# riktor/safer2-recommender

Hardware: AMD Instinct MI355X
Metric: user-solve updates/sec + sec/epoch, iALS dim=256 ml20m-shaped (higher is better)
Workload: dtype f32

## Files before the change

### safer2-recommender_amd/csrc/common.h

```cpp
#pragma once

#include <hip/hip_runtime.h>
#include <stdint.h>

#ifdef FRECSYS_ABLATION
#define FRECSYS_SKIP(mask, bit) ((mask) & (bit))
#else
#define FRECSYS_SKIP(mask, bit) 0
#endif

namespace frecsys_hip {

typedef float f32x16 __attribute__((ext_vector_type(16)));

enum {
  KIND_IALS = 0,
  KIND_WEIGHTED_U = 1,
  KIND_WEIGHTED_V = 2,
  KIND_CVAR_GRAD_U = 3,
  KIND_CVAR_GRAD_V = 4,
};

__host__ __device__ __forceinline__ bool is_v_kind(int k) {
  return k == KIND_WEIGHTED_V || k == KIND_CVAR_GRAD_V;
}
__host__ __device__ __forceinline__ bool is_u_kind(int k) {
  return k == KIND_WEIGHTED_U || k == KIND_CVAR_GRAD_U;
}
__host__ __device__ __forceinline__ bool is_grad_kind(int k) {
  return k == KIND_CVAR_GRAD_U || k == KIND_CVAR_GRAD_V;
}

__host__ __device__ constexpr int tidx(int I, int J) { return I * (I + 1) / 2 + J; }

__device__ __forceinline__ int sw(int r, int c) {
  return r * 32 + ((((c >> 2) ^ (r >> 1)) & 7) << 2) + (c & 3);
}
typedef float f32x4v __attribute__((ext_vector_type(4)));
__device__ __forceinline__ f32x4v row_gran(const float* tile, int r, int G) {
  return *reinterpret_cast<const f32x4v*>(tile + r * 32 + (((G ^ (r >> 1)) & 7) << 2));
}

__device__ __forceinline__ int acc_row(int q, int hi) {
  return (q & 3) + 8 * (q >> 2) + 4 * hi;
}

__device__ __forceinline__ void lds_barrier() {
  asm volatile("s_waitcnt lgkmcnt(0)" ::: "memory");
  __builtin_amdgcn_s_barrier();
  asm volatile("" ::: "memory");
}

__device__ __forceinline__ void wave_lds_sync() {
  asm volatile("s_waitcnt lgkmcnt(0)" ::: "memory");
  __builtin_amdgcn_wave_barrier();
  asm volatile("" ::: "memory");
}

__device__ __forceinline__ void glds16(const void* src, unsigned dst) {
  unsigned keep;
  asm volatile(
      "s_mov_b32 %0, m0\n\ts_mov_b32 m0, %2\n\ts_nop 0\n\t"
      "global_load_lds_dwordx4 %1, off\n\ts_mov_b32 m0, %0"
      : "=&s"(keep)
      : "v"(src), "s"(dst)
      : "memory");
}
__device__ __forceinline__ void glds4(const void* src, unsigned dst) {
  unsigned keep;
  asm volatile(
      "s_mov_b32 %0, m0\n\ts_mov_b32 m0, %2\n\ts_nop 0\n\t"
      "global_load_lds_dword %1, off\n\ts_mov_b32 m0, %0"
      : "=&s"(keep)
      : "v"(src), "s"(dst)
      : "memory");
}
__device__ __forceinline__ void vm_wait(int n) {
  switch (__builtin_amdgcn_readfirstlane(n)) {
    case 0: asm volatile("s_waitcnt vmcnt(0)" ::: "memory"); break;
    case 1: asm volatile("s_waitcnt vmcnt(1)" ::: "memory"); break;
    case 2: asm volatile("s_waitcnt vmcnt(2)" ::: "memory"); break;
    case 5: asm volatile("s_waitcnt vmcnt(5)" ::: "memory"); break;
    case 6: asm volatile("s_waitcnt vmcnt(6)" ::: "memory"); break;
    case 7: asm volatile("s_waitcnt vmcnt(7)" ::: "memory"); break;
    case 8: asm volatile("s_waitcnt vmcnt(8)" ::: "memory"); break;
    case 10: asm volatile("s_waitcnt vmcnt(10)" ::: "memory"); break;
    case 24: asm volatile("s_waitcnt vmcnt(24)" ::: "memory"); break;
    case 48: asm volatile("s_waitcnt vmcnt(48)" ::: "memory"); break;
    default: asm volatile("s_waitcnt vmcnt(0)" ::: "memory"); break;
  }
}
__device__ __forceinline__ void w3_barrier() {
  asm volatile("s_waitcnt lgkmcnt(0)" ::: "memory");
  __builtin_amdgcn_s_barrier();
  asm volatile("" ::: "memory");
}

__device__ __forceinline__ unsigned lds_addr(const void* p) {
  return (unsigned)(uintptr_t)(const __attribute__((address_space(3))) char*)p;
}

__device__ __forceinline__ f32x16 mfma32(float a, float b, f32x16 c) {
  return __builtin_amdgcn_mfma_f32_32x32x2f32(a, b, c, 0, 0, 0);
}

__device__ __forceinline__ uint32_t score_key(float x) {
  const uint32_t u = __float_as_uint(x);
  return (u & 0x80000000u) ? ~u : (u | 0x80000000u);
}
__device__ __forceinline__ float score_unkey(uint32_t key) {
  return __uint_as_float((key & 0x80000000u) ? (key ^ 0x80000000u) : ~key);
}

typedef __bf16 bf16x8 __attribute__((ext_vector_type(8)));

__device__ __forceinline__ void split3(float x, __bf16& h, __bf16& m, __bf16& l) {
  h = (__bf16)x;
  float r = x - (float)h;
  m = (__bf16)r;
  r -= (float)m;
  l = (__bf16)r;
}

__device__ __forceinline__ f32x16 mfma_bf16(bf16x8 a, bf16x8 b, f32x16 c) {
  return __builtin_amdgcn_mfma_f32_32x32x16_bf16(a, b, c, 0, 0, 0);
}

__device__ __forceinline__ f32x16 mfma_x6(const bf16x8 (&a)[3], const bf16x8 (&b)[3], f32x16 c) {
  c = mfma_bf16(a[2], b[0], c);
  c = mfma_bf16(a[0], b[2], c);
  c = mfma_bf16(a[1], b[1], c);
  c = mfma_bf16(a[1], b[0], c);
  c = mfma_bf16(a[0], b[1], c);
  c = mfma_bf16(a[0], b[0], c);
  return c;
}

__device__ __forceinline__ f32x16 mfma_x6s(const bf16x8 (&a)[3], const bf16x8 (&b)[3], f32x16 c) {
  c = mfma_bf16(a[0], b[0], c);
  c = mfma_bf16(a[0], b[1], c);
  c = mfma_bf16(a[1], b[0], c);
  c = mfma_bf16(a[0], b[2], c);
  c = mfma_bf16(a[1], b[1], c);
  c = mfma_bf16(a[2], b[0], c);
  return c;
}

__device__ __forceinline__ void split3x8(const float (&x)[8], bf16x8 (&f)[3]) {
#pragma unroll
  for (int j = 0; j < 8; ++j) {
    __bf16 h, m, l;
    split3(x[j], h, m, l);
    f[0][j] = h;
    f[1][j] = m;
    f[2][j] = l;
  }
}

__device__ __forceinline__ float entity_lambda(int kind, float reg, float reg_exp, float w,
                                               float alpha, int64_t h, int64_t n_other,
                                               const float* entity_reg, int64_t e,
// ... 107 lines not shown
```

### safer2-recommender_amd/csrc/dual.hip

```cpp
#include <hip/hip_runtime.h>

#include <cstdlib>
#include <type_traits>

#include "chol.h"
#include "common.h"
#include "kernels.h"

namespace frecsys_hip {

namespace {

constexpr int kMaxDp = 1024;

template <int HP>
__device__ __forceinline__ int dgran(int p, int g, int hh, int j) {
  return ((p * 2 + g) * 2 + hh) * HP + j;
}

template <int TH, bool BF>
struct DualCfg {
  static constexpr int HP = 32 * TH;
  static constexpr int NT = TH * (TH + 1) / 2;
  static constexpr int NW = (TH <= 4) ? 4 : 8;
  static constexpr int NTHR = NW * 64;
  static constexpr int MT = (NT + NW - 1) / NW;
  static constexpr int SROW = 33;
  static constexpr int STG = HP * SROW;
  static constexpr int ZS = (BF ? 48 : 32) * HP;
  static constexpr int TILES = NT * 1024;
  static constexpr int NSTAGE = BF ? 0 : ((TH <= 4) ? 1 : 2);
  static constexpr int NSTG1 = NSTAGE > 0 ? NSTAGE : 1;
  static constexpr int LOOP = ((NSTAGE * STG + ZS + 3) / 4) * 4;
  static constexpr int REGION0 = TILES > LOOP ? TILES : LOOP;
  static constexpr int OFF_C = REGION0;
  static constexpr int OFF_ID = OFF_C + HP;
  static constexpr int OFF_B = OFF_ID + HP;
  static constexpr int OFF_X = OFF_B + HP;
  static constexpr int PART = NTHR > NW * 32 ? NTHR : NW * 32;
  static constexpr int OFF_PART = OFF_X + HP;
  static constexpr int OFF_FLAG = OFF_PART + PART;
  static constexpr int OFF_L = OFF_FLAG + 4;
  static constexpr int NQ = (HP * 8 + NTHR - 1) / NTHR;
  static constexpr int WPE = (TH == 3 || TH == 5) ? 4 : (TH == 4 ? 3 : 1);
  static constexpr size_t bytes(int Dp) { return (size_t)(OFF_L + 2 * Dp) * 4; }
  static_assert(bytes(kMaxDp) <= 163840, "LDS budget");
};

__device__ __forceinline__ int64_t virt_pos_d(int64_t k, int64_t h) {
  return k < h ? k : (h - 128 + (k - h));
}

__device__ __forceinline__ void dual_scalars(const DualArgs& a, int64_t e, int64_t h, float& mu,
                                             float& lam, float& omega) {
  const int kind = a.kind;
  const bool uk = is_u_kind(kind);
  omega = (uk && a.entity_weight) ? a.entity_weight[e] : 1.0f;
  lam = entity_lambda(kind, a.reg, a.reg_exp, a.w, a.alpha, h, a.n_other, a.entity_reg, e,
                      a.lambda_is_reg);
  mu = uk ? omega * a.w : a.w;
}

__global__ void __launch_bounds__(256) dual_ldl_kernel(DualArgs a) {
  __shared__ float td[kMaxDp], to[kMaxDp];
  const int Dp = a.Dp, tid = threadIdx.x;
  if (a.unit_m) {
    const int64_t p = (int64_t)blockIdx.x * 256 + tid;
    if (p >= a.n_rows) return;
    const int64_t pp = a.pos0 + p;
    for (int k = 0; k < Dp; ++k) {
      a.table[blk_t(pp, 0, k, Dp)] = 0.0f;
      a.table[blk_t(pp, 1, k, Dp)] = 1.0f;
      a.table[blk_t(pp, 2, k, Dp)] = 1.0f;
    }
    if (!(a.basis_status[0] > 0.5f)) atomicMin(a.fail, (unsigned long long)(a.order[p].entity + 1));
    return;
  }
  for (int k = tid; k < Dp; k += 256) {
    td[k] = a.tdiag[k];
    to[k] = a.toff[k];
  }
  lds_barrier();
  const int64_t p = (int64_t)blockIdx.x * 256 + tid;
  if (p >= a.n_rows) return;
  const QueueRec rec = a.order[p];
  float mu, lam, omega;
  dual_scalars(a, rec.entity, rec.h, mu, lam, omega);
  const int64_t pp = a.pos0 + p;
  float r = 0.0f;
  bool ok = true;
  for (int k = 0; k < Dp; ++k) {
    const float b = k > 0 ? mu * to[k - 1] : 0.0f;
    const float l = b * r;
    const float dk = (mu * td[k] + lam) - l * b;
    ok = ok && (dk > 0.0f);
    r = __builtin_amdgcn_rcpf(dk);
    a.table[blk_t(pp, 0, k, Dp)] = l;
    a.table[blk_t(pp, 1, k, Dp)] = __builtin_amdgcn_rsqf(dk);
    a.table[blk_t(pp, 2, k, Dp)] = r;
  }
  if (!ok) atomicMin(a.fail, (unsigned long long)(rec.entity + 1));
}

constexpr int SWEEP_CH = 32;
__global__ void __launch_bounds__(256) dual_sweep_kernel(DualArgs a) {
  const int Dp = a.Dp;
  const int64_t p = (int64_t)blockIdx.x * 256 + threadIdx.x;
  if (p >= a.n_rows) return;
  const int64_t pp = a.pos0 + p;
  float u = 0.0f;
  for (int k0 = 0; k0 < Dp; k0 += SWEEP_CH) {
    float vv[SWEEP_CH], ll[SWEEP_CH], dd[SWEEP_CH];
#pragma unroll
    for (int j = 0; j < SWEEP_CH; ++j) {
      vv[j] = a.out_rot[blk_v(pp, k0 + j, Dp)];
      ll[j] = a.table[blk_t(pp, 0, k0 + j, Dp)];
      dd[j] = a.table[blk_t(pp, 2, k0 + j, Dp)];
    }
#pragma unroll
    for (int j = 0; j < SWEEP_CH; ++j) {
      u = vv[j] - ll[j] * u;
      a.out_rot[blk_v(pp, k0 + j, Dp)] = u * dd[j];
    }
  }
  float x = 0.0f;
  for (int k1 = Dp; k1 > 0; k1 -= SWEEP_CH) {
    float vv[SWEEP_CH], ll[SWEEP_CH];
#pragma unroll
    for (int j = 0; j < SWEEP_CH; ++j) {
      const int k = k1 - 1 - j;
      vv[j] = a.out_rot[blk_v(pp, k, Dp)];
      ll[j] = k + 1 < Dp ? a.table[blk_t(pp, 0, k + 1, Dp)] : 0.0f;
    }
#pragma unroll
    for (int j = 0; j < SWEEP_CH; ++j) {
      x = vv[j] - ll[j] * x;
      a.out_rot[blk_v(pp, k1 - 1 - j, Dp)] = x;
    }
  }
}

constexpr int kDualBlkTH = 3;

template <int TH, bool BF>
__global__ void __launch_bounds__((DualCfg<TH, BF>::NTHR))
    __attribute__((amdgpu_waves_per_eu(DualCfg<TH, BF>::WPE, 8))) dual_solve_kernel(DualArgs a) {
  using C = DualCfg<TH, BF>;
  constexpr bool RDS = BF;
  constexpr int HP = C::HP, NT = C::NT, NW = C::NW, NTHR = C::NTHR, MT = C::MT;
  constexpr int SROW = C::SROW, NQ = C::NQ;
  extern __shared__ __attribute__((aligned(16))) float smem[];
  float* tiles = smem;
  float* stage = smem;
  float* zs = smem + C::NSTAGE * C::STG;
  float* lsub = smem + C::OFF_L;
  float* dsq = lsub + a.Dp;
  float* cvec = smem + C::OFF_C;
  int* ids = reinterpret_cast<int*>(smem + C::OFF_ID);
  float* bvec = smem + C::OFF_B;
  float* xvec = smem + C::OFF_X;
  float* part = smem + C::OFF_PART;
  int* flag = reinterpret_cast<int*>(smem + C::OFF_FLAG);

  const int tid = threadIdx.x, lane = tid & 63;
  const int wave = __builtin_amdgcn_readfirstlane(tid >> 6);
  const int lo = lane & 31, hi = lane >> 5;
  const int kind = a.kind;
  const bool vk = is_v_kind(kind), uk = is_u_kind(kind);
  const int Dp = a.Dp, NC = Dp >> 5;

  const QueueRec rec = a.order[blockIdx.x];
  const int64_t e = rec.entity;
  const int64_t h = rec.h;
  const int64_t p0 = rec.p0;
  int64_t extra = 0;
  if (vk && a.quirk && h > 128 && (h % 128) != 0) extra = 128 - (h % 128);
  const int ntot = (int)(h + extra);

  const float hf = (float)h;
  float mu, lam, omega;
  dual_scalars(a, e, h, mu, lam, omega);
  (void)mu;
  (void)lam;

  int my_id = -1;
  if (tid < HP) {
    int id = -1;
    float cj = 0.0f;
    if (tid < ntot) {
      id = a.col[p0 + virt_pos_d(tid, h)];
      cj = vk ? sqrtf(a.other_weight[id]) : (uk ? sqrtf(omega / hf) : 1.0f);
    }
    ids[tid] = id;
    cvec[tid] = cj;
    bvec[tid] = tid < h ? cj : 0.0f;
    my_id = id;
  }
  if (tid == 0) flag[0] = 0;
  unsigned long long t_prev = a.prof ? clock64() : 0;
  auto mark = [&](int ph) {
    if (a.prof && tid == 0) {
      const unsigned long long t = clock64();
      atomicAdd(a.prof + ph, t - t_prev);
      t_prev = t;
    }
  };
  {
    const int64_t pp = a.pos0 + blockIdx.x;
    for (int k = tid; k < Dp; k += NTHR) {
      lsub[k] = FRECSYS_SKIP(a.debug_skip, 256) ? 0.5f : a.table[blk_t(pp, 0, k, Dp)];
      dsq[k] = FRECSYS_SKIP(a.debug_skip, 256) ? 0.5f : a.table[blk_t(pp, 1, k, Dp)];
    }
  }
  lds_barrier();

  float4 ra[NQ], rb[NQ];
  auto load_slab = [&](int c, float4 (&regs)[NQ]) {
#pragma unroll
    for (int q = 0; q < NQ; ++q) {
      const int s = tid + q * NTHR;
      if ((HP * 8) % NTHR == 0 || s < HP * 8) {
        const int r = s >> 3, c4 = s & 7;
        const int id = max(ids[r], 0);
        regs[q] = *reinterpret_cast<const float4*>(a.Xrot + (int64_t)id * Dp + 32 * c + 4 * c4);
      }
    }
  };
  auto store_slab = [&](const float4 (&regs)[NQ], int buf) {
#pragma unroll
    for (int q = 0; q < NQ; ++q) {
      const int s = tid + q * NTHR;
      if ((HP * 8) % NTHR == 0 || s < HP * 8) {
        const int r = s >> 3, c4 = s & 7;
        const bool ok = ids[r] >= 0 && !FRECSYS_SKIP(a.debug_skip, 32);
        float* d = stage + (buf % C::NSTG1) * C::STG + r * SROW + 4 * c4;
        d[0] = ok ? regs[q].x : 0.0f;
        d[1] = ok ? regs[q].y : 0.0f;
        d[2] = ok ? regs[q].z : 0.0f;
        d[3] = ok ? regs[q].w : 0.0f;
      }
    }
  };

  const float* myrow = a.Xrot + (int64_t)max(my_id, 0) * Dp;
  float4 yq[RDS ? 8 : 1];
  if constexpr (RDS) {
    if (tid < HP) {
#pragma unroll
      for (int q = 0; q < 8; ++q) yq[q] = *reinterpret_cast<const float4*>(myrow + 4 * q);
    }
  } else {
    load_slab(0, ra);
    if (NC > 1) load_slab(1, rb);
    store_slab(ra, 0);
  }
  lds_barrier();
  mark(0);

  f32x16 acc[MT];
  int aoff[MT], boff[MT];
  bool valid[MT];
#pragma unroll
  for (int m = 0; m < MT; ++m) {
    const int t = wave + m * NW;
    valid[m] = t < NT;
    int I = 0;
    while ((I + 1) * (I + 2) / 2 <= t) ++I;
    const int J = t - I * (I + 1) / 2;
    aoff[m] = 32 * I + lo;
    boff[m] = 32 * J + lo;
    acc[m] = f32x16{0.f};
  }
  float carry = 0.0f;
  const float cj = tid < HP ? cvec[tid] : 0.0f;
  auto slab_step = [&](int c, float4 (&mine)[NQ], float4 (&next)[NQ]) {
    if (!RDS && c + 2 < NC) load_slab(c + 2, mine);
    if (RDS && tid < HP && !FRECSYS_SKIP(a.debug_skip, 128)) {
      bf16x8* zb = reinterpret_cast<bf16x8*>(zs);
      float z = carry;
#pragma unroll
      for (int gh = 0; gh < 4; ++gh) {
        float v[8];
#pragma unroll
        for (int u = 0; u < 8; ++u) {
          const float4 y4 = yq[2 * gh + (u >> 2)];
          const float yv = (u & 3) == 0 ? y4.x : (u & 3) == 1 ? y4.y : (u & 3) == 2 ? y4.z : y4.w;
          const int k = 32 * c + 8 * gh + u;
          z = yv - lsub[k] * z;
          v[u] = (cj * z) * dsq[k];
        }
        if (c + 1 < NC) {
          yq[2 * gh] = *reinterpret_cast<const float4*>(myrow + 32 * (c + 1) + 8 * gh);
          yq[2 * gh + 1] = *reinterpret_cast<const float4*>(myrow + 32 * (c + 1) + 8 * gh + 4);
        }
        bf16x8 f[3];
        split3x8(v, f);
#pragma unroll
        for (int p = 0; p < 3; ++p) zb[dgran<HP>(p, gh >> 1, gh & 1, tid)] = f[p];
      }
      carry = z;
    }
    if (!RDS && tid < HP && !FRECSYS_SKIP(a.debug_skip, 128)) {
      const float* yrow = stage + ((c & 1) % C::NSTG1) * C::STG + tid * SROW;
      float y[BF ? 1 : 32];
      if constexpr (!BF) {
#pragma unroll
        for (int kk = 0; kk < 32; ++kk) y[kk] = yrow[kk];
      }
      float z = carry;
      if constexpr (BF) {
        bf16x8* zb = reinterpret_cast<bf16x8*>(zs);
#pragma unroll
        for (int gh = 0; gh < 4; ++gh) {
          float v[8];
#pragma unroll
          for (int u = 0; u < 8; ++u) {
            const int kk = 8 * gh + u, k = 32 * c + kk;
            z = yrow[kk] - lsub[k] * z;
            v[u] = (cj * z) * dsq[k];
          }
          bf16x8 f[3];
          split3x8(v, f);
#pragma unroll
          for (int p = 0; p < 3; ++p) zb[dgran<HP>(p, gh >> 1, gh & 1, tid)] = f[p];
        }
      } else {
#pragma unroll
        for (int kk = 0; kk < 32; ++kk) {
          const int k = 32 * c + kk;
          z = y[kk] - lsub[k] * z;
          zs[kk * HP + tid] = (cj * z) * dsq[k];
        }
      }
      carry = z;
    }
    lds_barrier();
    if (!FRECSYS_SKIP(a.debug_skip, 1)) {
      if constexpr (BF) {
        const bf16x8* zb = reinterpret_cast<const bf16x8*>(zs);
#pragma unroll
        for (int m = 0; m < MT; ++m) {
          if (valid[m]) {
#pragma unroll
            for (int g = 0; g < 2; ++g) {
              bf16x8 av[3], bv[3];
#pragma unroll
              for (int p = 0; p < 3; ++p) {
                av[p] = zb[dgran<HP>(p, g, hi, aoff[m])];
                bv[p] = zb[dgran<HP>(p, g, hi, boff[m])];
              }
              acc[m] = mfma_x6(av, bv, acc[m]);
            }
          }
        }
      } else {
#pragma unroll
        for (int m = 0; m < MT; ++m) {
          if (valid[m]) {
#pragma unroll
            for (int s = 0; s < 16; ++s) {
              const float* zr = zs + (2 * s + hi) * HP;
              acc[m] = mfma32(zr[aoff[m]], zr[boff[m]], acc[m]);
            }
          }
        }
      }
    }
    if (!RDS && c + 1 < NC) store_slab(next, (c + 1) & 1);
    lds_barrier();
  };
  for (int c = 0; c < NC; c += 2) {
    slab_step(c, ra, rb);
    if (c + 1 < NC) slab_step(c + 1, rb, ra);
  }

#pragma unroll
  for (int m = 0; m < MT; ++m) {
    if (valid[m]) {
      const int I = (aoff[m] - lo) >> 5, J = (boff[m] - lo) >> 5;
      float* tile = tiles + tidx(I, J) * 1024;
#pragma unroll
      for (int q = 0; q < 16; ++q) {
        const int i = acc_row(q, hi);
        const bool dg = (32 * I + i) == (32 * J + lo);
        tile[sw(i, lo)] = acc[m][q] + (dg ? 1.0f : 0.0f);
      }
    }
  }
  lds_barrier();
  mark(1);
  chol_solve_df<TH, NW, (TH >= kDualBlkTH)>(tiles, bvec, xvec, part, flag, tid, a.debug_skip,
                                            a.chol_sched != 0, a.prof);
  mark(2);

  {
    const int D4 = Dp >> 2, R = NTHR / D4;
    const int c4 = tid % D4, g = tid / D4;
    float* red = tiles;
    float4 acc4 = make_float4(0.f, 0.f, 0.f, 0.f);
    if (g < R && !FRECSYS_SKIP(a.debug_skip, 64)) {
      for (int j0 = g; j0 < ntot; j0 += 8 * R) {
        float4 rv[8];
        float wv[8];
#pragma unroll
        for (int u = 0; u < 8; ++u) {
          const int j = j0 + u * R;
          rv[u] = make_float4(0.f, 0.f, 0.f, 0.f);
          wv[u] = 0.0f;
          if (j < ntot) {
            wv[u] = cvec[j] * xvec[j];
            rv[u] = *reinterpret_cast<const float4*>(a.Xrot + (int64_t)ids[j] * Dp + 4 * c4);
          }
        }
#pragma unroll
        for (int u = 0; u < 8; ++u) {
          acc4.x += wv[u] * rv[u].x;
          acc4.y += wv[u] * rv[u].y;
          acc4.z += wv[u] * rv[u].z;
          acc4.w += wv[u] * rv[u].w;
        }
      }
      *reinterpret_cast<float4*>(red + g * Dp + 4 * c4) = acc4;
    }
    lds_barrier();
    for (int i = tid; i < Dp; i += NTHR) {
      float v = 0.0f;
      for (int gg = 0; gg < R; ++gg) v += red[gg * Dp + i];
      a.out_rot[blk_v(a.pos0 + blockIdx.x, i, Dp)] = v;
    }
  }
  mark(3);
  if (a.prof && tid == 0) atomicAdd(a.prof + 4, 1ull);
  if (tid == 0 && flag[0]) atomicMin(a.fail, (unsigned long long)(e + 1));
}


__device__ __forceinline__ void wave_sync() { wave_lds_sync(); }

template <int T>
__device__ __forceinline__ void chol_solve_wave(float* tiles, float* bvec, float* xvec,
                                                int* flag, int lane, int debug_skip) {
  const int lo = lane & 31, hi = lane >> 5;
  float y[T];
#pragma unroll
  for (int p = 0; p < T; ++p) {
    float* Tpp = tiles + tidx(p, p) * 1024;
    if (!FRECSYS_SKIP(debug_skip, 2) && !diag_factor_inv<true>(Tpp, lane) && lane == 0)
      flag[0] = 1;
    wave_sync();
    float yp = 0.0f;
#pragma unroll
    for (int g = 0; g < 8; ++g) {
      const f32x4v x4 = row_gran(Tpp, lo, g);
#pragma unroll
      for (int t = 0; t < 4; ++t) yp += x4[t] * bvec[32 * p + 4 * g + t];
    }
    y[p] = yp;
    if (hi == 0) xvec[32 * p + lo] = yp;
    if (p + 1 < T) {
      float* A10 = tiles + tidx(p + 1, p) * 1024;
      const f32x16 u = tile_pqT_x6(A10, Tpp, lo, hi);
      wave_sync();
#pragma unroll
      for (int q = 0; q < 16; ++q) A10[sw(acc_row(q, hi), lo)] = u[q];
      wave_sync();
      float t = 0.0f;
#pragma unroll
      for (int g = 0; g < 8; ++g) {
        const f32x4v x4 = row_gran(A10, lo, g);
#pragma unroll
        for (int u = 0; u < 4; ++u) t += x4[u] * xvec[32 * p + 4 * g + u];
      }
      const f32x16 w = tile_pqT_x6<true>(A10, A10, lo, hi);
      float* A11 = tiles + tidx(p + 1, p + 1) * 1024;
      wave_sync();
      if (hi == 0) bvec[32 * (p + 1) + lo] -= t;
#pragma unroll
      for (int q = 0; q < 16; ++q) A11[sw(acc_row(q, hi), lo)] -= w[q];
      wave_sync();
    }
  }
  float x1 = 0.0f;
  if (T == 2) {
    const float* T11 = tiles + tidx(1, 1) * 1024;
    float x = 0.0f;
#pragma unroll
    for (int i = 0; i < 32; ++i) x += T11[sw(i, lo)] * rdlane(y[1], i);
    x1 = x;
    if (hi == 0) xvec[32 + lo] = x;
    wave_sync();
  }
// ... 664 lines not shown
```

### safer2-recommender_amd/csrc/solve.hip

```cpp
#include <hip/hip_runtime.h>

#include <type_traits>

#include "chol.h"
#include "common.h"
#include "kernels.h"

constexpr int kSyrkSB = 1;

namespace frecsys_hip {

namespace {

constexpr int kRing = 4;

template <int T, bool BF>
struct TiledCfg {
  static constexpr int Dp = 32 * T;
  static constexpr int NT = T * (T + 1) / 2;
  static constexpr int NW = (T <= 2) ? 4 : 8;
  static constexpr int NTHR = NW * 64;
  static constexpr int MT = (NT + NW - 1) / NW;
  static constexpr int R = BF ? 32 : ((T <= 2) ? 16 : (T >= 8 ? 64 : 32));
  static constexpr int NSLOT = R * Dp / 4;
  static constexpr int NQ = (NSLOT + NTHR - 1) / NTHR;
  static constexpr int GRAN = 12 * Dp;
  static constexpr int TILES = NT * 1024;
  static constexpr int STAGE = BF ? 2 * 4 * GRAN : 2 * R * Dp;
  static constexpr int REGION0 = TILES > STAGE ? TILES : STAGE;
  static constexpr int OFF_B = REGION0;
  static constexpr int OFF_X = OFF_B + Dp;
  static constexpr int OFF_LD = OFF_X + Dp;
  static constexpr int OFF_SA = OFF_LD + 1024;
  static constexpr int OFF_BW = OFF_SA + kRing * R;
  static constexpr int OFF_ID = OFF_BW + kRing * R;
  static constexpr int OFF_FLAG = OFF_ID + kRing * R;
  static constexpr int TOTAL = OFF_FLAG + 4;
  static constexpr size_t BYTES = (size_t)TOTAL * 4;
  static_assert(BYTES <= 163840, "LDS budget");
  static_assert(R % 2 == 0, "row pairs");
  static_assert(!BF || 2 * Dp <= NTHR, "BF: one thread per (column, row group)");
};

template <int Dp>
__device__ __forceinline__ int bf_gran(int p, int g, int hh, int c) {
  return ((p * 2 + g) * 2 + hh) * Dp + c;
}

struct SbPat {
  int n, pa[5], pb[5];
};
__device__ constexpr SbPat kSbPat[5] = {
    {5, {0, 0, 1, 1, 1}, {2, 3, 2, 3, 0}},
    {4, {0, 0, 1, 1, 0}, {2, 3, 2, 3, 0}},
    {5, {0, 0, 1, 1, 0}, {2, 3, 2, 3, 0}},
    {4, {0, 1, 1, 2, 0}, {0, 0, 1, 2, 0}},
    {4, {0, 1, 2, 3, 0}, {0, 1, 2, 3, 0}},
};
__device__ __forceinline__ int sb_pattern(int wave) {
  constexpr int pat[8] = {0, 0, 2, 0, 1, 1, 3, 4};
  return pat[wave];
}
__device__ __forceinline__ int sb_block(int wave, int x) {
  constexpr int blk[8][4] = {{2, 3, 0, 1}, {4, 5, 0, 1}, {4, 5, 2, 3}, {6, 7, 0, 1},
                             {6, 7, 2, 3}, {6, 7, 4, 5}, {0, 1, 2, 2}, {3, 5, 6, 7}};
  return blk[wave][x];
}

__device__ __forceinline__ int64_t virt_pos(int64_t k, int64_t h) {
  return k < h ? k : (h - 128 + (k - h));
}

template <int T, bool PARTIAL, bool BF, bool OFF64 = false>
__global__ void __launch_bounds__((TiledCfg<T, BF>::NTHR))
    solve_tiled_kernel(SolveArgs a) {
  using C = TiledCfg<T, BF>;
  constexpr bool SB = BF && T == 8 && (kSyrkSB >= 2 || (PARTIAL && kSyrkSB >= 1));
  constexpr int Dp = C::Dp, NT = C::NT, NW = C::NW, NTHR = C::NTHR;
  constexpr int MT = C::MT;
  constexpr int R = C::R, NQ = C::NQ, NSLOT = C::NSLOT;
  extern __shared__ __attribute__((aligned(16))) float smem[];
  float* tiles = smem;
  float* stage = smem;
  float* bvec = smem + C::OFF_B;
  float* xvec = smem + C::OFF_X;
  float* part = smem + C::OFF_LD;
  float* ring_sa = smem + C::OFF_SA;
  float* ring_bw = smem + C::OFF_BW;
  int* ring_id = reinterpret_cast<int*>(smem + C::OFF_ID);
  int* flag = reinterpret_cast<int*>(smem + C::OFF_FLAG);

  const int tid = threadIdx.x, lane = tid & 63;
  const int wave = __builtin_amdgcn_readfirstlane(tid >> 6);
  const int lo = lane & 31, hi = lane >> 5;
  const int kind = a.kind;
  const bool vk = is_v_kind(kind);

  int qpos = blockIdx.x;
  int64_t k0 = 0, k1 = 0;
  int slab0 = 0, nslab = 0;
  if (PARTIAL) {
    const SplitWork wk = a.work[blockIdx.x];
    qpos = wk.pos;
    k0 = wk.k0;
    k1 = wk.k1;
    slab0 = wk.slab;
  } else if (qpos < a.n_split) {
    const int2 sp = a.split[qpos];
    slab0 = sp.x;
    nslab = sp.y;
  }
  const QueueRec rec = a.order[qpos];
  const int64_t e = rec.entity;
  const int64_t h = rec.h;
  const int64_t p0 = rec.p0;
  if (h == 0) return;
  int64_t extra = 0;
  if (vk && a.quirk && h > 128 && (h % 128) != 0) extra = 128 - (h % 128);
  const int64_t ntot = h + extra;
  if (!PARTIAL) k1 = nslab > 0 ? 0 : ntot;
  const int nchunks = (int)((k1 - k0 + R - 1) / R);

  auto ring_load = [&](int c, int& id, float& sa, float& bw) {
    const int64_t k = k0 + (int64_t)c * R + tid;
    id = -1;
    sa = 0.0f;
    bw = 0.0f;
    if (k < k1) {
      id = a.col[p0 + virt_pos(k, h)];
      if (vk) {
        const float nu = a.other_weight[id];
        sa = sqrtf(nu);
        bw = (k < h && sa > 0.0f) ? nu / sa : 0.0f;
      } else {
        sa = 1.0f;
        bw = 1.0f;
      }
    }
  };
  auto ring_id_load = [&](int c) {
    const int64_t k = k0 + (int64_t)c * R + tid;
    return k < k1 ? a.col[p0 + virt_pos(k, h)] : -1;
  };
  auto ring_store = [&](int c, int id, float sa, float bw) {
    const int s = (c % kRing) * R + tid;
    ring_id[s] = id;
    ring_sa[s] = sa;
    ring_bw[s] = bw;
  };
  const int bc = tid % Dp;
  const bool bown = BF && tid < 2 * Dp;
  const int bg = bown ? tid / Dp : 0;
  float bpart = 0.0f;
  auto load_bf = [&](int c, float (&xr)[16]) {
    if constexpr (BF) {
      const int4* ids = reinterpret_cast<const int4*>(ring_id + (c % kRing) * R + 16 * bg);
#pragma unroll
      for (int q = 0; q < 4; ++q) {
        const int4 id4 = ids[q];
        const int id[4] = {id4.x, id4.y, id4.z, id4.w};
#pragma unroll
        for (int j = 0; j < 4; ++j) {
          if constexpr (OFF64)
            xr[4 * q + j] = a.X[(int64_t)max(id[j], 0) * Dp + bc];
          else
            xr[4 * q + j] = a.X[(unsigned)max(id[j], 0) * (unsigned)Dp + (unsigned)bc];
        }
      }
    }
  };
  auto split_bf = [&](int c, const float (&xr)[16], bf16x8 (&f)[2][3], bool live) {
    if constexpr (BF) {
      const int base = (c % kRing) * R + 16 * bg;
      float sa[16], bw[16];
#pragma unroll
      for (int q = 0; q < 4; ++q) {
        const float4 s4 = reinterpret_cast<const float4*>(ring_sa + base)[q];
        const float4 w4 = reinterpret_cast<const float4*>(ring_bw + base)[q];
        sa[4 * q] = s4.x, sa[4 * q + 1] = s4.y, sa[4 * q + 2] = s4.z, sa[4 * q + 3] = s4.w;
        bw[4 * q] = w4.x, bw[4 * q + 1] = w4.y, bw[4 * q + 2] = w4.z, bw[4 * q + 3] = w4.w;
      }
      float bsum = 0.0f;
#pragma unroll
      for (int hh = 0; hh < 2; ++hh) {
        float v[8];
#pragma unroll
        for (int j = 0; j < 8; ++j) {
          const float x = xr[8 * hh + j] * sa[8 * hh + j];
          bsum += bw[8 * hh + j] * x;
          v[j] = x;
        }
        split3x8(v, f[hh]);
      }
      bpart = live ? bpart + bsum : bpart;
    }
  };
  auto scale_bf = [&](int c, const float (&xr)[16], float (&xs)[16], bool live) {
    if constexpr (BF) {
      const int base = (c % kRing) * R + 16 * bg;
      float bsum = 0.0f;
#pragma unroll
      for (int q = 0; q < 4; ++q) {
        const float4 s4 = reinterpret_cast<const float4*>(ring_sa + base)[q];
        const float4 w4 = reinterpret_cast<const float4*>(ring_bw + base)[q];
        const float sa[4] = {s4.x, s4.y, s4.z, s4.w}, bw[4] = {w4.x, w4.y, w4.z, w4.w};
#pragma unroll
        for (int j = 0; j < 4; ++j) {
          xs[4 * q + j] = xr[4 * q + j] * sa[j];
          bsum += bw[j] * xs[4 * q + j];
        }
      }
      bpart = live ? bpart + bsum : bpart;
    }
  };
  auto write_bf = [&](int buf, const bf16x8 (&f)[2][3]) {
    if constexpr (BF) {
      bf16x8* st = reinterpret_cast<bf16x8*>(stage) + buf * C::GRAN;
      if (bown) {
#pragma unroll
        for (int hh = 0; hh < 2; ++hh)
#pragma unroll
          for (int p = 0; p < 3; ++p) st[bf_gran<Dp>(p, bg, hh, bc)] = f[hh][p];
      }
    }
  };
  constexpr int NQR = BF ? 1 : NQ;
  float4 regs[NQR];
  auto load_data = [&](int c) {
    {
      const int slot = c % kRing;
#pragma unroll
      for (int q = 0; q < NQR; ++q) {
        const int sidx = tid + q * NTHR;
        regs[q] = make_float4(0.f, 0.f, 0.f, 0.f);
        if (NSLOT % NTHR == 0 || sidx < NSLOT) {
          const int r = sidx / (Dp / 4), c4 = sidx % (Dp / 4);
          const int id = ring_id[slot * R + r];
          if (id >= 0) regs[q] = *reinterpret_cast<const float4*>(a.X + (int64_t)id * Dp + 4 * c4);
        }
      }
    }
  };
  auto store_stage = [&](int buf, int c) {
    {
      float* st = stage + buf * R * Dp;
      const int slot = c % kRing;
#pragma unroll
      for (int q = 0; q < NQR; ++q) {
        const int sidx = tid + q * NTHR;
        if (NSLOT % NTHR == 0 || sidx < NSLOT) {
          float4 v = regs[q];
          if (vk) {
            const float sc = ring_sa[slot * R + sidx / (Dp / 4)];
            v.x *= sc;
            v.y *= sc;
            v.z *= sc;
            v.w *= sc;
          }
          *reinterpret_cast<float4*>(st + 4 * sidx) = v;
        }
      }
    }
  };

  if (tid == 0) flag[0] = 0;
  unsigned long long t_prev = (!PARTIAL && a.prof) ? clock64() : 0;
  auto mark = [&](int ph) {
    if (!PARTIAL && a.prof && tid == 0) {
      const unsigned long long t = clock64();
      atomicAdd(a.prof + ph, t - t_prev);
      t_prev = t;
    }
  };
  if (tid < R) {
#pragma unroll
    for (int c = 0; c < (BF ? 3 : 2); ++c) {
      if (c < nchunks) {
        int id;
        float sa, bw;
        ring_load(c, id, sa, bw);
        ring_store(c, id, sa, bw);
      }
    }
  }
  if (!PARTIAL && is_grad_kind(kind) && tid < Dp) xvec[tid] = a.E[e * Dp + tid];

  const float hf = (float)h;
  const float omega = (is_u_kind(kind) && a.entity_weight) ? a.entity_weight[e] : 1.0f;
  const float lam =
      entity_lambda(kind, a.reg, a.reg_exp, a.w, a.alpha, h, a.n_other, a.entity_reg, e,
                    a.lambda_is_reg);
  const bool grad = is_grad_kind(kind);
  const float gscale = kind == KIND_IALS ? a.w : (is_u_kind(kind) ? hf * a.w : a.w);
  const float lam_d = kind == KIND_IALS ? lam : 0.0f;
  f32x16 acc[MT];
  int aoff[MT], boff[MT];
  bool valid[MT];
#pragma unroll
  for (int m = 0; m < MT; ++m) {
    int I = 0, J = 0;
    if constexpr (SB) {
      const SbPat& pt = kSbPat[sb_pattern(wave)];
      valid[m] = m < pt.n;
      I = sb_block(wave, pt.pa[m]);
      J = sb_block(wave, pt.pb[m]);
    } else {
      const int t = wave + m * NW;
      valid[m] = t < NT;
      while ((I + 1) * (I + 2) / 2 <= t) ++I;
      J = t - I * (I + 1) / 2;
    }
    aoff[m] = 32 * I + lo;
    boff[m] = 32 * J + lo;
    acc[m] = f32x16{0.f};
    if (!PARTIAL && valid[m] && !grad) {
#pragma unroll
      for (int q = 0; q < 16; ++q) {
        const int gi = 32 * I + acc_row(q, hi), gj = 32 * J + lo;
        acc[m][q] = gscale * a.G[gi * Dp + gj] + (gi == gj ? lam_d : 0.0f);
      }
    }
  }
  int sbx[4] = {0, 0, 0, 0};
  if constexpr (SB) {
#pragma unroll
    for (int x = 0; x < 4; ++x) sbx[x] = sb_block(wave, x);
  }
  float bacc = 0.0f;
  const size_t slab_floats = (size_t)NT * 1024 + Dp;
  for (int sidx = 0; sidx < nslab; ++sidx) {
    const float* sl = a.slabs + (size_t)(slab0 + sidx) * slab_floats;
#pragma unroll
    for (int m = 0; m < MT; ++m) {
      if (valid[m]) {
        const int t = tidx((aoff[m] - lo) >> 5, (boff[m] - lo) >> 5);
#pragma unroll
        for (int q = 0; q < 16; ++q) acc[m][q] += sl[t * 1024 + q * 64 + lane];
      }
    }
    if (tid < Dp) bacc += sl[NT * 1024 + tid];
  }
  const float us = omega / hf;
  auto write_tiles = [&](auto mode_c) __attribute__((always_inline)) {
    constexpr int MODE = decltype(mode_c)::value;
#pragma unroll
    for (int m = 0; m < MT; ++m) {
      if (valid[m]) {
        const int I = (aoff[m] - lo) >> 5, J = (boff[m] - lo) >> 5;
        float* tile = tiles + tidx(I, J) * 1024;
#pragma unroll
        for (int q = 0; q < 16; ++q) {
          const int i = acc_row(q, hi);
          const bool dg = (32 * I + i) == (32 * J + lo);
          float v = acc[m][q];
          if constexpr (MODE == 1) v = v * us + (dg ? lam : 0.0f);
          if constexpr (MODE == 2) v = v + (dg ? lam : 0.0f);
          if constexpr (MODE == 3)
            v = assemble(kind, v, a.G[(32 * I + i) * Dp + 32 * J + lo], dg, a.w, lam, hf, omega);
          tile[sw(i, lo)] = v;
        }
      }
    }
  };
  auto store_tiles = [&]() __attribute__((always_inline)) {
    if constexpr (PARTIAL) {
      float* sl = a.slabs + (size_t)slab0 * slab_floats;
#pragma unroll
      for (int m = 0; m < MT; ++m) {
        if (valid[m]) {
          const int t = tidx((aoff[m] - lo) >> 5, (boff[m] - lo) >> 5);
#pragma unroll
          for (int q = 0; q < 16; ++q) sl[t * 1024 + q * 64 + lane] = acc[m][q];
        }
      }
    } else {
      if (grad) write_tiles(std::integral_constant<int, 3>{});
      else if (is_u_kind(kind)) write_tiles(std::integral_constant<int, 1>{});
      else if (vk) write_tiles(std::integral_constant<int, 2>{});
      else write_tiles(std::integral_constant<int, 0>{});
    }
  };
  lds_barrier();
  mark(0);
  if constexpr (BF) {
    float xa[16], xb[16];
    if (nchunks > 0) {
      load_bf(0, xa);
      bf16x8 f[2][3];
      split_bf(0, xa, f, true);
      write_bf(0, f);
    }
    if (nchunks > 1) load_bf(1, xa);
    lds_barrier();
    float wpend = 0.0f;
    auto step = [&](int c, float (&xcur)[16], float (&xnxt)[16], auto pc)
                    __attribute__((always_inline)) {
      const int buf = c & 1;
      const bool ring_more = (tid < R) && (c + 3 < nchunks);
      int nid = -1;
      if (ring_more) nid = ring_id_load(c + 3);
      load_bf(c + 2 < nchunks ? c + 2 : nchunks - 1, xnxt);
      const bool live = c + 1 < nchunks;
      float xs[16];
      scale_bf(c + 1, xcur, xs, live);
      bf16x8 f[2][3];
      constexpr int SLOTS = (NT / NW) * 2 > 0 ? (NT / NW) * 2 : 1;
      constexpr int PER = (16 + SLOTS - 1) / SLOTS;
      auto split_slot = [&](int slot) {
#pragma unroll
        for (int u = 0; u < PER; ++u) {
          const int j = slot * PER + u;
          if (j < 16) {
            __bf16 h, m, l;
            split3(xs[j], h, m, l);
            f[j >> 3][0][j & 7] = h;
            f[j >> 3][1][j & 7] = m;
            f[j >> 3][2][j & 7] = l;
          }
        }
#pragma unroll
        for (int hh = 0; hh < 2; ++hh)
          if ((slot * PER) >> 3 == hh || (slot * PER + PER - 1) >> 3 == hh)
#pragma unroll
            for (int p = 0; p < 3; ++p) asm volatile("" : "+v"(f[hh][p]));
      };
      const bf16x8* st = reinterpret_cast<const bf16x8*>(stage) + buf * C::GRAN;
      if (SB && !FRECSYS_SKIP(a.debug_skip, 1)) {
        {
          constexpr SbPat P = kSbPat[decltype(pc)::value];
          constexpr int NX = decltype(pc)::value == 3 ? 3 : 4;
#pragma unroll
          for (int g = 0; g < 2; ++g) {
            bf16x8 fr[NX][3];
#pragma unroll
            for (int x = 0; x < NX; ++x)
#pragma unroll
              for (int p = 0; p < 3; ++p) fr[x][p] = st[bf_gran<Dp>(p, g, hi, 32 * sbx[x] + lo)];
#pragma unroll
            for (int m = 0; m < P.n; ++m) {
              acc[m] = mfma_x6s(fr[P.pa[m]], fr[P.pb[m]], acc[m]);
              if (m < 4) split_slot(4 * g + m);
            }
          }
        }
      } else if (!FRECSYS_SKIP(a.debug_skip, 1)) {
#pragma unroll
        for (int m = 0; m < MT; ++m) {
          if (m < NT / NW || valid[m]) {
#pragma unroll
            for (int g = 0; g < 2; ++g) {
              bf16x8 av[3], bv[3];
#pragma unroll
              for (int p = 0; p < 3; ++p) {
                av[p] = st[bf_gran<Dp>(p, g, hi, aoff[m])];
                bv[p] = st[bf_gran<Dp>(p, g, hi, boff[m])];
              }
              acc[m] = mfma_x6s(av, bv, acc[m]);
              if (m < NT / NW) split_slot(2 * m + g);
            }
          }
        }
        if constexpr (NT / NW == 0) split_slot(0);
      } else {
#pragma unroll
        for (int k = 0; k < SLOTS; ++k) split_slot(k);
      }
      if (live) write_bf(buf ^ 1, f);
      if (tid < R && c >= 1 && c + 2 < nchunks) {
        const int64_t k = k0 + (int64_t)(c + 2) * R + tid;
        float sa = 0.0f, bw = 0.0f;
        if (k < k1) {
          if (vk) {
            sa = sqrtf(wpend);
            bw = (k < h && sa > 0.0f) ? wpend / sa : 0.0f;
          } else {
            sa = 1.0f;
            bw = 1.0f;
          }
        }
        const int s = ((c + 2) % kRing) * R + tid;
        ring_sa[s] = sa;
        ring_bw[s] = bw;
      }
      if (ring_more) {
        ring_id[((c + 3) % kRing) * R + tid] = nid;
        if (vk) wpend = a.other_weight[max(nid, 0)];
      }
      lds_barrier();
    };
    auto loop = [&](auto pc) __attribute__((always_inline)) {
      for (int c = 0; c < nchunks; c += 2) {
        step(c, xa, xb, pc);
        if (c + 1 < nchunks) step(c + 1, xb, xa, pc);
      }
      store_tiles();
    };
    if constexpr (SB) {
      switch (sb_pattern(wave)) {
        case 0: loop(std::integral_constant<int, 0>{}); break;
        case 1: loop(std::integral_constant<int, 1>{}); break;
        case 2: loop(std::integral_constant<int, 2>{}); break;
        case 3: loop(std::integral_constant<int, 3>{}); break;
        default: loop(std::integral_constant<int, 4>{}); break;
      }
    } else {
      loop(std::integral_constant<int, 0>{});
    }
  } else {
    if (nchunks > 0) {
      load_data(0);
      store_stage(0, 0);
    }
    lds_barrier();
    for (int c = 0; c < nchunks; ++c) {
      const int buf = c & 1;
      const bool more = c + 1 < nchunks;
      const bool ring_more = (tid < R) && (c + 2 < nchunks);
      if (more) load_data(c + 1);
      int nid = -1;
      float nsa = 0.f, nbw = 0.f;
      if (ring_more) ring_load(c + 2, nid, nsa, nbw);
      const float* st = stage + buf * R * Dp;
      const int slot = c % kRing;
      if (!FRECSYS_SKIP(a.debug_skip, 1)) {
#pragma unroll
        for (int m = 0; m < MT; ++m) {
          if (valid[m]) {
#pragma unroll
            for (int s = 0; s < R / 2; ++s) {
              const float* rowp = st + (2 * s + hi) * Dp;
              acc[m] = mfma32(rowp[aoff[m]], rowp[boff[m]], acc[m]);
            }
          }
        }
      }
      if (tid < Dp) {
#pragma unroll 4
        for (int r = 0; r < R; ++r) bacc += ring_bw[slot * R + r] * st[r * Dp + tid];
      }
      if (more) store_stage(buf ^ 1, c + 1);
      if (ring_more) ring_store(c + 2, nid, nsa, nbw);
      lds_barrier();
    }
    store_tiles();
  }
  mark(1);
  if constexpr (BF) {
    if (bown && bg == 1) part[bc] = bpart;
    lds_barrier();
    if (tid < Dp) bacc += bpart + part[tid];
    lds_barrier();
  }
  mark(9);

  if (PARTIAL) {
    if (tid < Dp) a.slabs[(size_t)slab0 * slab_floats + NT * 1024 + tid] = bacc;
    return;
  }

  mark(10);
  if (tid < Dp) {
    float b = bacc;
    if (is_u_kind(kind)) b *= us;
    bvec[tid] = b;
  }
  lds_barrier();
  mark(2);

  if (grad) {
    if (tid < Dp) {
      const int i = tid, I = i >> 5, ri = i & 31;
      float y = 0.0f;
      for (int j = 0; j < Dp; ++j) {
        float aij;
        if (j <= i)
          aij = tiles[tidx(I, j >> 5) * 1024 + sw(ri, j & 31)];
        else
          aij = cvar_upper(kind, a.G[i * Dp + j], a.w, omega);
        y += aij * xvec[j];
      }
      a.out[e * Dp + i] = xvec[i] - a.eta * (y - bvec[i]);
    }
    return;
  }

  chol_solve_df<T, NW>(tiles, bvec, xvec, part, flag, tid, a.debug_skip, a.chol_sched != 0,
                       a.prof);
  mark(3);
  if (tid < Dp) a.out[e * Dp + tid] = xvec[tid];
  if (tid == 0 && flag[0]) atomicMin(a.fail, (unsigned long long)(e + 1));
  if (a.prof && tid == 0) {
    atomicAdd(a.prof + 4, 1ull);
    atomicAdd(a.prof + 8, (unsigned long long)ntot);
  }
}

__device__ __forceinline__ void wave_sync() {
  __builtin_amdgcn_fence(__ATOMIC_RELEASE, "wavefront");
  __builtin_amdgcn_wave_barrier();
  __builtin_amdgcn_fence(__ATOMIC_ACQUIRE, "wavefront");
}

template <int Dp>
__global__ void __launch_bounds__(256) solve_small_kernel(SolveArgs a) {
  constexpr int WPB = 4, CH = 64, PER = Dp * Dp / 64;
  __shared__ float sA[WPB][Dp * Dp];
  __shared__ float sX[WPB][CH * Dp];
  __shared__ float sB[WPB][Dp];
  __shared__ float sE[WPB][Dp];
  __shared__ float sSA[WPB][CH];
  __shared__ float sBW[WPB][CH];
  const int wave = threadIdx.x >> 6, lane = threadIdx.x & 63;
  const int64_t idx = (int64_t)blockIdx.x * WPB + wave;
  if (idx >= a.n_rows) return;
  const int64_t e = a.row_lo + idx;
  const int64_t p0 = a.row_ptr[e];
  const int64_t h = a.row_ptr[e + 1] - p0;
  if (h == 0) return;
  const int kind = a.kind;
  const bool vk = is_v_kind(kind);
  int64_t extra = 0;
  if (vk && a.quirk && h > 128 && (h % 128) != 0) extra = 128 - (h % 128);
  const int64_t ntot = h + extra;
  float acc[PER];
#pragma unroll
  for (int t = 0; t < PER; ++t) acc[t] = 0.0f;
  float bacc = 0.0f;
  float* X = sX[wave];
  for (int64_t c0 = 0; c0 < ntot; c0 += CH) {
    const int64_t k = c0 + lane;
    int id = -1;
    float sa = 0.f, bw = 0.f;
    if (k < ntot) {
      id = a.col[p0 + virt_pos(k, h)];
      if (vk) {
        const float nu = a.other_weight[id];
        sa = sqrtf(nu);
        bw = (k < h) ? nu : 0.0f;
      } else {
        sa = 1.0f;
        bw = 1.0f;
      }
    }
    sSA[wave][lane] = sa;
    sBW[wave][lane] = bw;
#pragma unroll
// ... 203 lines not shown
```

Baseline: 9.664 million.

## Software-pipeline bf16 SYRK fragment loads with MFMA and overlap next-chunk gather

In the tiled solve kernel (T=8, non-SB bf16 path), LDS fragment loads for the next MFMA tile are double-buffered and issued ahead of the current MFMA, with sched_barriers enforcing order. The global gather and scaling for the next chunk are moved inside the MFMA loop so memory latency overlaps compute, and half of the split staging is written early. The dual solve kernel gets a similar prefetch of fragments for TH=4/6. This costs more registers, carries occupancy risk, and makes scheduling brittle.

```diff
diff --git a/safer2-recommender_amd/csrc/common.h b/safer2-recommender_amd/csrc/common.h
--- a/safer2-recommender_amd/csrc/common.h
+++ b/safer2-recommender_amd/csrc/common.h
@@ -7,6 +7,10 @@
 #define FRECSYS_SKIP(mask, bit) ((mask) & (bit))
 #else
 #define FRECSYS_SKIP(mask, bit) 0
+#endif
+
+#ifndef FRECSYS_SYRK_PIPE
+#define FRECSYS_SYRK_PIPE 1
 #endif
 
 namespace frecsys_hip {
diff --git a/safer2-recommender_amd/csrc/dual.hip b/safer2-recommender_amd/csrc/dual.hip
--- a/safer2-recommender_amd/csrc/dual.hip
+++ b/safer2-recommender_amd/csrc/dual.hip
@@ -149,6 +149,8 @@
   constexpr bool RDS = BF;
   constexpr int HP = C::HP, NT = C::NT, NW = C::NW, NTHR = C::NTHR, MT = C::MT;
   constexpr int SROW = C::SROW, NQ = C::NQ;
+  constexpr int PF = !(FRECSYS_SYRK_PIPE && BF) ? 0 : (TH == 4 || TH == 6) ? 3 : 0;
+  static_assert(PF == 0 || NW <= NT, "PF: every wave owns a first tile");
   extern __shared__ __attribute__((aligned(16))) float smem[];
   float* tiles = smem;
   float* stage = smem;
@@ -336,7 +338,34 @@
     }
     lds_barrier();
     if (!FRECSYS_SKIP(a.debug_skip, 1)) {
-      if constexpr (BF) {
+      if constexpr (BF && PF > 0) {
+        const bf16x8* zb = reinterpret_cast<const bf16x8*>(zs);
+        auto frag = [&](int k, bool early, bf16x8 (&av)[3], bf16x8 (&bv)[3]) {
+          const int m = k >> 1, g = k & 1;
+          if (early) {
+            av[2] = zb[dgran<HP>(2, g, hi, aoff[m])];
+            bv[0] = zb[dgran<HP>(0, g, hi, boff[m])];
+            av[0] = zb[dgran<HP>(0, g, hi, aoff[m])];
+          }
+          if (early == (PF == 6)) {
+            bv[2] = zb[dgran<HP>(2, g, hi, boff[m])];
+            av[1] = zb[dgran<HP>(1, g, hi, aoff[m])];
+            bv[1] = zb[dgran<HP>(1, g, hi, boff[m])];
+          }
+        };
+        bf16x8 fa[2][3], fb[2][3];
+        frag(0, true, fa[0], fb[0]);
+#pragma unroll
+        for (int k = 0; k < 2 * MT; ++k) {
+          if (valid[k >> 1]) {
+            if (PF < 6) frag(k, false, fa[k & 1], fb[k & 1]);
+            if (k + 1 < 2 * MT && valid[(k + 1) >> 1])
+              frag(k + 1, true, fa[(k + 1) & 1], fb[(k + 1) & 1]);
+            __builtin_amdgcn_sched_barrier(0);
+            acc[k >> 1] = mfma_x6(fa[k & 1], fb[k & 1], acc[k >> 1]);
+          }
+        }
+      } else if constexpr (BF) {
         const bf16x8* zb = reinterpret_cast<const bf16x8*>(zs);
 #pragma unroll
         for (int m = 0; m < MT; ++m) {
diff --git a/safer2-recommender_amd/csrc/solve.hip b/safer2-recommender_amd/csrc/solve.hip
--- a/safer2-recommender_amd/csrc/solve.hip
+++ b/safer2-recommender_amd/csrc/solve.hip
@@ -76,6 +76,7 @@
     solve_tiled_kernel(SolveArgs a) {
   using C = TiledCfg<T, BF>;
   constexpr bool SB = BF && T == 8 && (kSyrkSB >= 2 || (PARTIAL && kSyrkSB >= 1));
+  constexpr bool PIPE = FRECSYS_SYRK_PIPE && BF && !SB && T == 8;
   constexpr int Dp = C::Dp, NT = C::NT, NW = C::NW, NTHR = C::NTHR;
   constexpr int MT = C::MT;
   constexpr int R = C::R, NQ = C::NQ, NSLOT = C::NSLOT;
@@ -213,12 +214,12 @@
       bpart = live ? bpart + bsum : bpart;
     }
   };
-  auto write_bf = [&](int buf, const bf16x8 (&f)[2][3]) {
+  auto write_bf = [&](int buf, const bf16x8 (&f)[2][3], int hh0 = 0) {
     if constexpr (BF) {
       bf16x8* st = reinterpret_cast<bf16x8*>(stage) + buf * C::GRAN;
       if (bown) {
 #pragma unroll
-        for (int hh = 0; hh < 2; ++hh)
+        for (int hh = hh0; hh < 2; ++hh)
 #pragma unroll
           for (int p = 0; p < 3; ++p) st[bf_gran<Dp>(p, bg, hh, bc)] = f[hh][p];
       }
@@ -399,10 +400,11 @@
       const bool ring_more = (tid < R) && (c + 3 < nchunks);
       int nid = -1;
       if (ring_more) nid = ring_id_load(c + 3);
-      load_bf(c + 2 < nchunks ? c + 2 : nchunks - 1, xnxt);
+      auto gather_next = [&]() { load_bf(c + 2 < nchunks ? c + 2 : nchunks - 1, xnxt); };
+      if constexpr (!PIPE) gather_next();
       const bool live = c + 1 < nchunks;
       float xs[16];
-      scale_bf(c + 1, xcur, xs, live);
+      if constexpr (!PIPE) scale_bf(c + 1, xcur, xs, live);
       bf16x8 f[2][3];
       constexpr int SLOTS = (NT / NW) * 2 > 0 ? (NT / NW) * 2 : 1;
       constexpr int PER = (16 + SLOTS - 1) / SLOTS;
@@ -424,8 +426,10 @@
 #pragma unroll
             for (int p = 0; p < 3; ++p) asm volatile("" : "+v"(f[hh][p]));
       };
-      const bf16x8* st = reinterpret_cast<const bf16x8*>(stage) + buf * C::GRAN;
-      if (SB && !FRECSYS_SKIP(a.debug_skip, 1)) {
+      int sbase = buf * C::GRAN;
+      if constexpr (PIPE) asm volatile("" : "+s"(sbase));
+      const bf16x8* st = reinterpret_cast<const bf16x8*>(stage) + sbase;
+      if (SB &&!FRECSYS_SKIP(a.debug_skip, 1)) {
         {
           constexpr SbPat P = kSbPat[decltype(pc)::value];
           constexpr int NX = decltype(pc)::value == 3 ? 3 : 4;
@@ -441,6 +445,45 @@
               acc[m] = mfma_x6s(fr[P.pa[m]], fr[P.pb[m]], acc[m]);
               if (m < 4) split_slot(4 * g + m);
             }
+          }
+        }
+      } else if (PIPE && !FRECSYS_SKIP(a.debug_skip, 1)) {
+        constexpr int FULL = NT / NW;
+        static_assert(!PIPE || (SLOTS == 2 * FULL && PER * SLOTS == 16 && 2 * Dp == NTHR),
+                      "PIPE: a slot per common group, every thread stages");
+        auto frag = [&](int m, int g, bf16x8 (&av)[3], bf16x8 (&bv)[3]) {
+#pragma unroll
+          for (int p = 0; p < 3; ++p) {
+            av[p] = st[bf_gran<Dp>(p, g, hi, aoff[m])];
+            bv[p] = st[bf_gran<Dp>(p, g, hi, boff[m])];
+          }
+        };
+        bf16x8 fa[2][3], fb[2][3];
+        if (MT > FULL && valid[MT - 1]) {
+          frag(MT - 1, 0, fa[0], fb[0]);
+          frag(MT - 1, 1, fa[1], fb[1]);
+          __builtin_amdgcn_sched_barrier(0);
+          acc[MT - 1] = mfma_x6s(fa[0], fb[0], acc[MT - 1]);
+          frag(0, 0, fa[0], fb[0]);
+          __builtin_amdgcn_sched_barrier(0);
+          acc[MT - 1] = mfma_x6s(fa[1], fb[1], acc[MT - 1]);
+        } else {
+          frag(0, 0, fa[0], fb[0]);
+        }
+        bf16x8* so = reinterpret_cast<bf16x8*>(stage) + (C::GRAN - sbase);
+#pragma unroll
+        for (int k = 0; k < 2 * FULL; ++k) {
+          if (k + 1 < 2 * FULL) frag((k + 1) >> 1, (k + 1) & 1, fa[(k + 1) & 1], fb[(k + 1) & 1]);
+          __builtin_amdgcn_sched_barrier(0);
+          acc[k >> 1] = mfma_x6s(fa[k & 1], fb[k & 1], acc[k >> 1]);
+          if (k == 0) {
+            gather_next();
+            scale_bf(c + 1, xcur, xs, live);
+          }
+          split_slot(k);
+          if (k == FULL - 1) {
+#pragma unroll
+            for (int p = 0; p < 3; ++p) so[bf_gran<Dp>(p, bg, 0, bc)] = f[0][p];
           }
         }
       } else if (!FRECSYS_SKIP(a.debug_skip, 1)) {
@@ -462,10 +505,14 @@
         }
         if constexpr (NT / NW == 0) split_slot(0);
       } else {
+        if constexpr (PIPE) {
+          gather_next();
+          scale_bf(c + 1, xcur, xs, live);
+        }
 #pragma unroll
         for (int k = 0; k < SLOTS; ++k) split_slot(k);
       }
-      if (live) write_bf(buf ^ 1, f);
+      if (live) write_bf(buf ^ 1, f, PIPE && !FRECSYS_SKIP(a.debug_skip, 1) ? 1 : 0);
       if (tid < R && c >= 1 && c + 2 < nchunks) {
         const int64_t k = k0 + (int64_t)(c + 2) * R + tid;
         float sa = 0.0f, bw = 0.0f;
@@ -489,9 +536,18 @@
       lds_barrier();
     };
     auto loop = [&](auto pc) __attribute__((always_inline)) {
-      for (int c = 0; c < nchunks; c += 2) {
-        step(c, xa, xb, pc);
-        if (c + 1 < nchunks) step(c + 1, xb, xa, pc);
+      if constexpr (PIPE) {
+        int c = 0;
+        for (; c + 1 < nchunks; c += 2) {
+          step(c, xa, xb, pc);
+          step(c + 1, xb, xa, pc);
+        }
+        if (c < nchunks) step(c, xa, xb, pc);
+      } else {
+        for (int c = 0; c < nchunks; c += 2) {
+          step(c, xa, xb, pc);
+          if (c + 1 < nchunks) step(c + 1, xb, xa, pc);
+        }
       }
       store_tiles();
     };
```

Result: faster. 9.770 million (median of 6 runs) (+1.1%).
